# hhergeth/CudaTracerLib

Measured on AMD Instinct MI355X. Metric: Mrays/s at 1920x1080, 267 spp (steps), depth-8; achieved HBM GB/s vs peak, higher is better.
Workload: dtype f32; 1 GPU; synthetic-SM 1920x1080, 1 spp/step, depth 8, NEE on, 2000 instances x icosphere(4)/boxes, 8631000 instanced triangles; rough_transmittance=the reference's 3-D lookup on every call (bit-equal frames), framebuffer_reduce=none (1 GPU)

## Files before the change

### cudatracerlib_amd/build.py

```python
import hashlib, os, subprocess, sys, glob, tempfile

HERE = os.path.dirname(os.path.abspath(__file__))
CSRC = os.path.join(HERE, "csrc")
OUT = os.path.join(HERE, "libctl_amd.so")
SRCS = ["kernels.hip", "shade_basic.hip", "shade_full.hip", "shade_class_a.hip", "shade_class_b.hip", "shade_class_c.hip", "shade_class_p.hip", "shade_class_g.hip", "shade_class_g_wf.hip", "shade_class_p_wf.hip", "shade_class_a_wf.hip", "shade_class_b_wf.hip", "shade_class_c_wf.hip", "shade_basic_wf.hip", "shade_full_wf.hip", "shade_full_media.hip", "shade_full_media_grid.hip", "shade_full_partials.hip", "medium_stage.hip", "megakernel.hip", "prim_tracer.hip", "traversal_probe.hip", "shading_eval_basic.hip", "shading_eval_full.hip", "shading_eval_partials.hip", "image_pipeline.hip", "nlm_filter.hip", "block_sampler.hip", "tracer.hip", "scene_update.hip", "flat_refit.hip", "flat_rebuild.hip", "flat_nodes.hip", "flat_meshes.hip", "flat_mesh_set.hip", "mesh_skin.hip", "shape_set.hip", "scene_images.hip", "volume_eval.hip", "capi.hip", "scene_builder.cpp", "scene_checks.cpp", "geometry_hash.cpp", "bvh_builder.cpp", "sbvh_builder.cpp", "flatten.cpp", "flat_rebuild.cpp", "flat_nodes.cpp", "flat_meshes.cpp", "flat_mesh_set.cpp", "mitsuba_loader.cpp", "image_io.cpp", "jpeg_decode.cpp", "mesh_io.cpp", "scene_cache.cpp", "comm.cpp"]
FLAGS = ["-O3", "-std=c++17", "--offload-arch=gfx950", "-fPIC", "-ffp-contract=off", "-munsafe-fp-atomics",
         "-Wall", "-Wno-unused-function", "-Wno-unused-variable", "-pthread",
         "-Xarch_device", "-fno-slp-vectorize"]


KNOBS_OUT = os.path.join(HERE, "libctl_knobs.so")


def _flag_key(defines=()):
    return hashlib.sha256(("\0".join(sorted(defines)) + "\1" + os.environ.get("CTL_BUILD_EXTRA_FLAGS", "")).encode()).hexdigest()[:16]


def _object_dir(out):
    if out is None:
        return os.path.join(HERE, "build")
    return os.path.join(os.environ.get("TMPDIR") or tempfile.gettempdir(), "ctl_build_" + os.path.splitext(os.path.basename(out))[0])


def stale(target=None, defines=()):
# ... 50 lines not shown
```

### cudatracerlib_amd/csrc/device_scene.h

```cpp
#pragma once
#include "../../include/ctl_amd.h"
#include "ctl_math.h"

namespace ctl {

constexpr int kExitMarker = 0x76543211;
enum { kShadeMoreBsdfs = 1, kShadeRoughBsdfs = 2, kShadeImageTextures = 4, kShadeMoreLights = 8, kShadeNestingBsdfs = 16, kShadeSurfaceMaps = 32, kShadeMoreMicrofacet = 64 };
constexpr int kStackSize = 96;

inline bool is_simple_bsdf(uint32_t t) {
    return t == CTL_BSDF_DIFFUSE || t == CTL_BSDF_DIELECTRIC || t == CTL_BSDF_THINDIELECTRIC || t == CTL_BSDF_ROUGHDIELECTRIC || t == CTL_BSDF_CONDUCTOR || t == CTL_BSDF_ROUGHCONDUCTOR ||
           t == CTL_BSDF_PLASTIC || t == CTL_BSDF_PHONG || t == CTL_BSDF_ROUGHDIFFUSE || t == CTL_BSDF_WARD || t == CTL_BSDF_ROUGHPLASTIC;
}
inline int nested_bsdf_count(uint32_t t) { return t == CTL_BSDF_BLEND ? 2 : (t == CTL_BSDF_COATING || t == CTL_BSDF_ROUGHCOATING) ? 1 : 0; }
inline bool is_nesting_bsdf(uint32_t t) { return nested_bsdf_count(t) != 0; }
inline const uint32_t* bsdf_distribution(const ctl_material& m) {
    const uint32_t t = m.bsdf_type;
    if (t == CTL_BSDF_ROUGHPLASTIC) return &m.u[2];
    return (t == CTL_BSDF_ROUGHCONDUCTOR || t == CTL_BSDF_ROUGHDIELECTRIC || t == CTL_BSDF_ROUGHCOATING) ? &m.u[0] : nullptr;
}
inline bool bsdf_reads_rough_transmittance(uint32_t t) { return t == CTL_BSDF_ROUGHPLASTIC || t == CTL_BSDF_ROUGHCOATING; }
inline uint32_t bsdf_shade_features(const ctl_material& m) {
    const uint32_t t = m.bsdf_type;
    uint32_t f = 0;
// ... 62 lines not shown
    const float* rt_reduced;
    int start_node;
    uint32_t n_nodes;
    uint32_t num_lights;
    uint32_t env_map_index;
    uint32_t n_lights_buf, n_anim_bytes, n_materials_probe;
    uint32_t alpha_maps;
    uint32_t shade_features;
    uint32_t shade_models;
    float eps;
    uint32_t light_indices[CTL_MAX_NUM_LIGHTS];
    float light_cdf[CTL_MAX_NUM_LIGHTS];
    dev_sensor cam;
};

}
```

### cudatracerlib_amd/csrc/kernels.h

```cpp
#pragma once
#include "device_scene.h"
#include "block_sampler.h"
#include <hip/hip_runtime.h>

namespace ctl {

namespace vol { struct table; }

struct path_soa {
    float4* ray_o;
    float4* ray_d;
    float4* thr;
    float4* rad;
    float4* nor;
    float4* pend;
    float2* px;
    float4* mrec;
};
enum { kFlagSpecular = 1 };
constexpr int kHitConsumed = -2;
constexpr uint32_t kNoShadow = 0xffffffffu;

struct final_soa {
    float4* rad;
// ... 29 lines not shown
    uint32_t n_local_pixels;
    int direct, max_path_length, rr_start_depth;
    int key_from_traversal;
    int model_classes;
    const unsigned char* block_counts;
    uint32_t max_block_count;
    int wavefront_rules;
    int u16_bary;
    float* debug_out; uint32_t debug_x, debug_y;
    float* depth_buffer; uint32_t depth_w, depth_h; float depth_near, depth_far;
    float4* stage; size_t stage_stride;
    float4* stray_stage;
    int tex_partials;
};

struct launch_ctx { hipStream_t stream; int grid_blocks; bool alpha_test = false; };

void launch_sequence_fill(hipStream_t stream, const uint32_t* jumps, const void* starts, uint32_t n_passes, float* t1, float* t2);

void apply_tuning_from_env();
void launch_raygen(const launch_ctx& lc, const dev_scene& S, const wave_queues& Q, const pass_params& P);
void launch_intersect_closest(const launch_ctx& lc, const dev_scene& S, const float4* ro, const float4* rd, const uint32_t* n_ptr, uint32_t* work, float4* hit, int* hit_node);
void launch_intersect_any(const launch_ctx& lc, const dev_scene& S, const float4* ro, const float4* rd, const uint32_t* n_ptr, uint32_t* work, uint32_t* occ, float4* hit = nullptr, int* hit_node = nullptr);
void launch_intersect_pair(const launch_ctx& lc, const dev_scene& S, const float4* ro, const float4* rd, const uint32_t* n_ptr, uint32_t* work, float4* hit, int* hit_node,
                           const float4* sro, const float4* srd, const uint32_t* sn_ptr, uint32_t* swork, uint32_t* occ);
void launch_intersect_count(const launch_ctx& lc, const dev_scene& S, const float4* ro, const float4* rd, const uint32_t* n_ptr, uint32_t* work, float4* hit, int* hit_node,
                            uint32_t* occ, int any_hit, unsigned long long* counts3);
void launch_shade(const launch_ctx& lc, const dev_scene& S, const wave_queues& Q, const pass_params& P, int depth, ctl_pixel_data* image, const vol::table* media = nullptr);
void read_stack_histogram(unsigned long long* h, bool reset);
#define CTL_SHADE_BUILDS(X) \
    X(basic, 0u) X(full, 0u) \
    X(class_a, 0u) X(class_b, CTL_CLASS_B_KEYS) X(class_g, CTL_CLASS_G_KEYS) X(class_p, CTL_CLASS_P_KEYS) X(class_c, CTL_CLASS_C_KEYS)
using shade_launch = void(const launch_ctx& lc, const dev_scene& S, const wave_queues& Q, const pass_params& P, int depth, ctl_pixel_data* image);
#define CTL_SHADE_DECLARE(name, keys) shade_launch launch_shade_##name, launch_shade_##name##_wf;
CTL_SHADE_BUILDS(CTL_SHADE_DECLARE)
#undef CTL_SHADE_DECLARE
using shade_media_launch = void(const launch_ctx& lc, const dev_scene& S, const wave_queues& Q, const pass_params& P, const vol::table& V, int depth, ctl_pixel_data* image);
// ... 26 lines not shown
```

### cudatracerlib_amd/csrc/kernels.hip

```cpp
#include "kernels.h"
#include "traverse.h"
#include "traverse_flat.h"
#include "traverse_flat8.h"
#include "knobs.h"
#include <stdexcept>
#include <type_traits>
#include "shading.h"
#include "compaction.h"
#include "volume.h"
#include <cstdlib>

namespace ctl {

__global__ __launch_bounds__(kWideBlock) void k_raygen(dev_scene S, wave_queues Q, pass_params P) {
    __shared__ uint32_t s_cnt[3][kWideBlock / 64]; __shared__ uint32_t s_base[3];
    const uint32_t tiles_x = (P.width + 63) / 64;
    const uint32_t n_total = P.n_local_pixels * P.batch;
    const uint32_t n1 = CTL_SAMPLER_NUM_SEQUENCES * CTL_SAMPLER_SEQUENCE_LENGTH;
    for (uint32_t gi = blockIdx.x * kWideBlock + threadIdx.x; gi < n_total; gi += gridDim.x * kWideBlock) {
        const uint32_t pass_b = gi / P.n_local_pixels, li = gi - pass_b * P.n_local_pixels;
        uint32_t x, y; const uint32_t tile = tile_order_pixel(tiles_x, P.tile_rank, P.tile_world, li, x, y);
        const uint32_t n_smp = P.block_counts ? P.block_counts[tile] : 1u, max_smp = P.block_counts ? P.max_block_count : 1u;
        for (uint32_t smp = 0; smp < max_smp; smp++) {
        const bool valid = x < P.width && y < P.height && smp < n_smp;
// ... 5 lines not shown
        const f2 pX{ (float)x + j.x, (float)y + j.y };
        const f2 ap = rng.next2();
        f3 o, d; sensor_sample_ray(S.cam, pX, ap, o, d);
        const path_soa& A = Q.path[0];
        A.ray_o[slot] = make_float4(o.x, o.y, o.z, S.eps);
        A.ray_d[slot] = make_float4(d.x, d.y, d.z, 3.402823466e+38f);
        A.thr[slot] = make_float4(1.0f, 1.0f, 1.0f, 0.0f);
        A.rad[slot] = make_float4(0.0f, 0.0f, 0.0f, __uint_as_float(pixel));
        A.nor[slot] = make_float4(0.0f, 0.0f, 0.0f, __uint_as_float(rng.d1 | (rng.d2 << 8) | (pass_b << 16) | (0u << 24)));
        A.pend[slot] = make_float4(0.0f, 0.0f, 0.0f, __uint_as_float(kNoShadow));
        A.px[slot] = make_float2(pX.x, pX.y);
        }
    }
}

#ifndef CTL_INTERSECT_MIN_WAVES
#define CTL_INTERSECT_MIN_WAVES 7
#endif
constexpr int lds_stack_ints(int layout) { return layout == 1 + kFmtQ8 ? (kQ8LdsRows + 1) * 2 * kBlock : (layout ? kFlatLdsRows + 1 : kLdsStack) * kBlock; }
template <bool ANY_HIT, bool COUNT, int LAYOUT, bool ALPHA>
__device__ __forceinline__ void intersect_flat_layout(const dev_scene& S, const float4* __restrict__ ro, const float4* __restrict__ rd, uint32_t n, uint32_t* __restrict__ work, float4* __restrict__ hit, int* __restrict__ hit_node, uint32_t* __restrict__ occ, int* lds_stack, trav_counts& tc) {
    if (LAYOUT == 1 + kFmtQ8) intersect_flat8<ANY_HIT, COUNT, ALPHA>(S, ro, rd, n, work, hit, hit_node, occ, (unsigned long long*)lds_stack, tc);
    else intersect_flat<ANY_HIT, COUNT, ALPHA>(S, ro, rd, n, work, hit, hit_node, occ, lds_stack, tc);
}
template <bool ANY_HIT, bool COUNT, int LAYOUT, bool ALPHA>
#ifdef CTL_INTERSECT_EXACT_WAVES
#define CTL_INTERSECT_WAVES_ATTR __attribute__((amdgpu_waves_per_eu(CTL_INTERSECT_EXACT_WAVES, CTL_INTERSECT_EXACT_WAVES)))
#else
#define CTL_INTERSECT_WAVES_ATTR
#endif
__global__ __launch_bounds__(kBlock, ((LAYOUT && !ALPHA) ? CTL_INTERSECT_MIN_WAVES : 6)) CTL_INTERSECT_WAVES_ATTR void k_intersect(dev_scene S, const float4* __restrict__ ro, const float4* __restrict__ rd, const uint32_t* __restrict__ n_ptr,
                                                       uint32_t* __restrict__ work, float4* __restrict__ hit, int* __restrict__ hit_node, uint32_t* __restrict__ occ,
                                                       unsigned long long* __restrict__ counts3) {
    __shared__ __attribute__((aligned(8))) int lds_stack[lds_stack_ints(LAYOUT)];
    const uint32_t n = *n_ptr;
    trav_counts tc{ 0, 0, 0, 0, 0 };
    if (LAYOUT) intersect_flat_layout<ANY_HIT, COUNT, LAYOUT, ALPHA>(S, ro, rd, n, work, hit, hit_node, occ, lds_stack, tc);
    else intersect_persistent<ANY_HIT, COUNT, ALPHA>(S, ro, rd, n, work, hit, hit_node, occ, lds_stack, tc);
    if (COUNT) {
        atomicAdd(&counts3[0], (unsigned long long)tc.n_inner); atomicAdd(&counts3[1], (unsigned long long)tc.n_tri); atomicAdd(&counts3[2], (unsigned long long)tc.n_inst);
        atomicAdd(&counts3[3], (unsigned long long)tc.w_inner); atomicAdd(&counts3[4], (unsigned long long)tc.w_tri);
    }
}

template <int LAYOUT, bool ALPHA>
// ... 127 lines not shown
    }
}

__global__ __launch_bounds__(kBlock) void k_add_samples(ctl_pixel_data* __restrict__ image, uint32_t W, uint32_t H, uint32_t n, const float* __restrict__ s) {
    for (uint32_t i = blockIdx.x * kBlock + threadIdx.x; i < n; i += gridDim.x * kBlock) add_sample(image, W, H, s[5 * i], s[5 * i + 1], f3(s[5 * i + 2], s[5 * i + 3], s[5 * i + 4]));
}
void launch_add_samples(const launch_ctx& lc, ctl_pixel_data* image, uint32_t W, uint32_t H, uint32_t n, const float* samples5) {
    hipLaunchKernelGGL(k_add_samples, dim3(lc.grid_blocks), dim3(kBlock), 0, lc.stream, image, W, H, n, samples5);
}

void read_stack_histogram(unsigned long long* h, bool reset) {
    if (hipMemcpyFromSymbol(h, HIP_SYMBOL(g_stack_hist), sizeof(unsigned long long) * kStackSize) != hipSuccess) throw std::runtime_error("reading the stack histogram failed");
    if (reset) { unsigned long long z[kStackSize] = {}; if (hipMemcpyToSymbol(HIP_SYMBOL(g_stack_hist), z, sizeof(z)) != hipSuccess) throw std::runtime_error("clearing the stack histogram failed"); }
}
static unsigned g_lds_pad = 0;
static int traversal_blocks(const launch_ctx& lc, int layout, bool alpha) {
    const int cus = lc.grid_blocks / 8, by_regs = (layout && !alpha) ? CTL_INTERSECT_MIN_WAVES : 6;
    const int by_lds = (int)((160u * 1024u) / ((unsigned)sizeof(int) * (unsigned)lds_stack_ints(layout) + g_lds_pad));
    return cus * (by_regs < by_lds ? by_regs : by_lds);
}
void apply_tuning_from_env() {
    static bool done = false;
    if (done) return;
    done = true;
    if (const char* e = knob_env("CTL_LDS_PAD")) { int v = atoi(e); if (v >= 0 && v <= 140000) g_lds_pad = (unsigned)v; }
    if (const char* e = knob_env("CTL_REFILL_IDLE")) { int v = atoi(e); if (v >= 1 && v <= 64) (void)hipMemcpyToSymbol(HIP_SYMBOL(g_refill_idle), &v, sizeof(v)); }
    if (const char* e = knob_env("CTL_CHUNK_GUIDED")) { int v = atoi(e) != 0; (void)hipMemcpyToSymbol(HIP_SYMBOL(g_chunk_guided), &v, sizeof(v)); }
    if (const char* e = knob_env("CTL_LEAF_BATCH")) { int v = atoi(e); if (v >= 1 && v <= 64) (void)hipMemcpyToSymbol(HIP_SYMBOL(g_leaf_batch), &v, sizeof(v)); }
    if (const char* e = knob_env("CTL_LEAF_BATCH_ANY")) { int v = atoi(e); if (v >= 1 && v <= 64) (void)hipMemcpyToSymbol(HIP_SYMBOL(g_leaf_batch_any), &v, sizeof(v)); }
}

void launch_raygen(const launch_ctx& lc, const dev_scene& S, const wave_queues& Q, const pass_params& P) {
    hipLaunchKernelGGL(k_raygen, dim3(lc.grid_blocks / 4), dim3(kWideBlock), 0, lc.stream, S, Q, P);
}
template <class F>
static void with_traversal_kernel(const launch_ctx& lc, const dev_scene& S, F&& f) {
    auto alpha = [&](auto layout) { if (lc.alpha_test) f(layout, std::true_type{}); else f(layout, std::false_type{}); };
    if (!S.flat_nodes) alpha(std::integral_constant<int, 0>{});
    else if (S.flat_format == kFmtQ8) alpha(std::integral_constant<int, 1 + kFmtQ8>{});
    else alpha(std::integral_constant<int, 1 + kFmtQ4>{});
}
template <bool ANY, bool CNT>
static void launch_intersect(const launch_ctx& lc, const dev_scene& S, const float4* ro, const float4* rd, const uint32_t* n_ptr, uint32_t* work, float4* hit, int* hit_node,
                             uint32_t* occ, unsigned long long* counts3) {
    with_traversal_kernel(lc, S, [&](auto layout, auto alpha) {
        constexpr int L = decltype(layout)::value; constexpr bool A = decltype(alpha)::value;
        hipLaunchKernelGGL((k_intersect<ANY, CNT, L, A>), dim3(traversal_blocks(lc, L, A)), dim3(kBlock), g_lds_pad, lc.stream, S, ro, rd, n_ptr, work, hit, hit_node, occ, counts3);
    });
}
void launch_intersect_closest(const launch_ctx& lc, const dev_scene& S, const float4* ro, const float4* rd, const uint32_t* n_ptr, uint32_t* work, float4* hit, int* hit_node) {
    launch_intersect<false, false>(lc, S, ro, rd, n_ptr, work, hit, hit_node, nullptr, nullptr);
}
void launch_intersect_any(const launch_ctx& lc, const dev_scene& S, const float4* ro, const float4* rd, const uint32_t* n_ptr, uint32_t* work, uint32_t* occ, float4* hit, int* hit_node) {
    launch_intersect<true, false>(lc, S, ro, rd, n_ptr, work, hit, hit_node, occ, nullptr);
}
void launch_intersect_pair(const launch_ctx& lc, const dev_scene& S, const float4* ro, const float4* rd, const uint32_t* n_ptr, uint32_t* work, float4* hit, int* hit_node,
                           const float4* sro, const float4* srd, const uint32_t* sn_ptr, uint32_t* swork, uint32_t* occ) {
    with_traversal_kernel(lc, S, [&](auto layout, auto alpha) {
        constexpr int L = decltype(layout)::value; constexpr bool A = decltype(alpha)::value;
        hipLaunchKernelGGL((k_intersect_pair<L, A>), dim3(traversal_blocks(lc, L, A)), dim3(kBlock), g_lds_pad, lc.stream, S, ro, rd, n_ptr, work, hit, hit_node, sro, srd, sn_ptr, swork, occ);
    });
}
void launch_intersect_count(const launch_ctx& lc, const dev_scene& S, const float4* ro, const float4* rd, const uint32_t* n_ptr, uint32_t* work, float4* hit, int* hit_node,
                            uint32_t* occ, int any_hit, unsigned long long* counts3) {
    if (any_hit) launch_intersect<true, true>(lc, S, ro, rd, n_ptr, work, hit, hit_node, occ, counts3);
    else launch_intersect<false, true>(lc, S, ro, rd, n_ptr, work, hit, hit_node, nullptr, counts3);
// ... 80 lines not shown
```

### cudatracerlib_amd/csrc/tracer.h

```cpp
#pragma once
#include "../../include/ctl_amd.h"
#include "device_scene.h"
#include "kernels.h"
#include "sequence_generator.h"
#include "block_sampler.h"
#include "flatten.h"
#include <hip/hip_runtime.h>
#include <map>
#include <set>
#include <string>
#include <vector>
#include <memory>
#include <stdexcept>
#include <climits>

namespace ctl {

struct hip_error : std::runtime_error { using std::runtime_error::runtime_error; };
void throw_hip(hipError_t e, const char* file, int line);
#define CTL_HIP(x) do { hipError_t _e = (x); if (_e != hipSuccess) ::ctl::throw_hip(_e, __FILE__, __LINE__); } while (0)

template <typename T> struct dbuf {
    T* p = nullptr; size_t n = 0;
    dbuf() {}
// ... 265 lines not shown
    void check_media(const Scene* s) const;
    void check_texture_filtering() const;
    void setDepthBuffer(float* device_data, unsigned int dw, unsigned int dh) override { depth_buffer_ = device_data; depth_w_ = dw; depth_h_ = dh; }
    void reservePasses(unsigned int n) override { const unsigned int b = std::min(passBatch(), std::max(1u, n)); growBatch(b, "reservePasses"); ensureTableRing(b); if (w != 0xffffffffu) (void)ensureStage(b); }
protected:
    void DoRender(Image* I, const float* d_t1, const float* d_t2, unsigned int n_batch) override;
    void takeRayCounts(uint64_t& path_rays, uint64_t& shadow_rays_) override;
    unsigned int passBatch() const override;
    bool updatesVarianceInBatch(unsigned int b) override;
private:
    void growBatch(unsigned int b, const char* who);
    float4* ensureStage(unsigned int b);
    wave_queues Q{};
    uint32_t capacity = 0, n_local_pixels = 0, alloc_batch_ = 1;
    float* depth_buffer_ = nullptr; unsigned int depth_w_ = 0, depth_h_ = 0;
    std::vector<std::unique_ptr<dbuf<float4>>> f4_; dbuf<float2> px_[2]; dbuf<float4> stage_, stray_stage_, mrec_[2]; dbuf<int> hit_node_; dbuf<uint32_t> occ_[2], counts_, work_, class_order_, class_counts_; dbuf<unsigned char> mat_key_; dbuf<unsigned long long> stats_;
    int grid_blocks = 0;
    float4* new_f4(size_t n);
};

class PathTracer : public Tracer<true> {
public:
    PathTracer();
    void Resize(unsigned int w, unsigned int h) override;
    void InitializeScene(Scene* s) override;
protected:
    void DoRender(Image* I, const float* d_t1, const float* d_t2, unsigned int n_batch) override;
    void takeRayCounts(uint64_t& path_rays, uint64_t& shadow_rays_) override;
    void DebugInternal(Image* I, unsigned int x, unsigned int y, const float* d_t1, const float* d_t2, float rgb[3]) override;
private:
    dbuf<float> debug_;
// ... 21 lines not shown
```

### cudatracerlib_amd/csrc/tracer.hip

```cpp
#include "tracer.h"
#include "scene_builder.h"
#include "scene_checks.h"
#include "scene_volumes.h"
#include "flatten.h"
#include "image_io.h"
#include "mitsuba_loader.h"
#include "spline.h"
#include "mip_pyramid.h"
#include "ctl_fmath.h"
#include "knobs.h"
#include <algorithm>
#include <thread>
#include <cctype>
#include <cstring>
#include <cstdlib>
#include <string>

namespace ctl {

void throw_hip(hipError_t e, const char* file, int line) {
    throw hip_error(std::string("In file ") + file + ", line " + std::to_string(line) + " : " + hipGetErrorString(e));
}
int device_count() { int n = 0; if (hipGetDeviceCount(&n) != hipSuccess) return 0; return n; }
void require_device() { if (device_count() <= 0) throw hip_error("no HIP device: the MI355X path tracer has no CPU fallback"); apply_tuning_from_env(); }
// ... 454 lines not shown
    takeRayCounts(intersect_rays, shadow_rays);
    m_uLastNumRaysTraced = intersect_rays + shadow_rays;
    m_fAccRuntime += m_fLastRuntime; m_uAccNumRaysTraced += m_uLastNumRaysTraced;
}
template class Tracer<true>;
template class Tracer<false>;

WavefrontPathTracer::WavefrontPathTracer() {
    m_sParameters.addBool("Direct", true);
    m_sParameters.addInterval("MaxPathLength", 50, 1, INT_MAX);
    m_sParameters.addInterval("RRStartDepth", 5, 1, INT_MAX);
    m_sParameters.addInterval("PassBatch", 0, 0, 128);
    m_sParameters.addBool("AlphaTest", false);
    m_sParameters.addBool("ShadeByModelClass", true);
    m_sParameters.addBool("FuseTraversal", true);
    m_sParameters.addEnum("PathSemantics", 0, { "PathTrace", "Wavefront" });
    m_sParameters.addBool("U16Barycentrics", false);
    m_sParameters.addInterval("OrderedAccumulationMaxMB", 4096, 0, 1 << 20);
    m_sParameters.addBool("ParticipatingMedia", false);
    m_sParameters.addBool("TextureFiltering", false);
    m_sParameters.addBool("OrderedAccumulation", true);
    grid_blocks = persistent_grid_blocks();
}
void WavefrontPathTracer::check_media(const Scene* s) const {
    if (m_sParameters.getValue("ParticipatingMedia") == 0) { if (s) s->refuse_volumes("WavefrontPathTracer"); return; }
    if (m_sParameters.getValue("PathSemantics") == 1)
        throw unsupported_error("WavefrontPathTracer: ParticipatingMedia = true with PathSemantics = Wavefront is not supported: pathIterateKernel has no medium rules; participating media are rendered under PathSemantics = PathTrace");
}
void WavefrontPathTracer::check_texture_filtering() const {
    if (m_sParameters.getValue("TextureFiltering") == 0) return;
// ... 101 lines not shown
    P.t1 = d_t1p; P.t2 = (const float2*)d_t2p;
    P.batch = n_batch;
    P.width = w; P.height = h; P.tile_rank = shard_rank; P.tile_world = shard_world; P.n_local_pixels = n_local_pixels;
    P.direct = direct ? 1 : 0; P.max_path_length = maxPathLength; P.rr_start_depth = rrStart;
    P.block_counts = pass_block_counts_; P.max_block_count = pass_max_block_count_;
    P.wavefront_rules = m_sParameters.getValue("PathSemantics") == 1 ? 1 : 0; P.u16_bary = m_sParameters.getValue("U16Barycentrics") != 0 ? 1 : 0;
    P.tex_partials = (m_sParameters.getValue("TextureFiltering") != 0 && (S.shade_features & kShadeImageTextures)) ? 1 : 0;
    P.depth_buffer = depth_buffer_; P.depth_w = depth_w_; P.depth_h = depth_h_; P.depth_near = m_pScene->near_depth; P.depth_far = m_pScene->far_depth;
    P.stage = nullptr; P.stage_stride = (size_t)n_local_pixels;
    if (!pass_block_counts_) P.stage = ensureStage(n_batch);
    P.stray_stage = (batch_variance_ && P.stage) ? stray_stage_.p : nullptr;
    if (pass_block_counts_ && pass_paths_ > capacity) throw std::runtime_error("ray queue overflow: the block sampler asks for more samples in one pass than the queues hold (DoubleRayBuffer.h:86-89)");
    CTL_HIP(hipMemsetAsync(class_counts_.p, 0, n_class * sizeof(uint32_t), stream));
    CTL_HIP(hipMemsetAsync(counts_.p, 0, n_counts * sizeof(uint32_t), stream));
    CTL_HIP(hipMemsetAsync(work_.p, 0, n_work * sizeof(uint32_t), stream));
    timer.begin(stream, 0); launch_raygen(lc, S, Q, P); timer.end(stream);
    auto shadow_pass = [&](int d) {
        timer.begin(stream, 3);
        if (counting) launch_intersect_count(lc, S, Q.sh_o[d & 1], Q.sh_d[d & 1], &Q.counts[d * 4 + 1], &Q.work[2 * d + 3], nullptr, nullptr, Q.sh_occ[d & 1], 1, Q.stats + 7);
        else launch_intersect_any(lc, S, Q.sh_o[d & 1], Q.sh_d[d & 1], &Q.counts[d * 4 + 1], &Q.work[2 * d + 3], Q.sh_occ[d & 1]);
        timer.end(stream);
        shadow_launches++;
    };
    const bool fuse = !counting && direct && m_sParameters.getValue("FuseTraversal") != 0;
    P.model_classes = (!media && S.shade_features != 0 && m_sParameters.getValue("ShadeByModelClass") != 0) ? 1 : 0;
    dev_scene Sk = S; Sk.hit_key_out = (!media && S.flat_leaf_keys && (S.shade_features == 0 || P.model_classes) && !counting) ? Q.mat_key : nullptr;
    P.key_from_traversal = Sk.hit_key_out ? 1 : 0;
    if (!P.key_from_traversal) P.model_classes = 0;
    if (P.model_classes && !class_order_.p) { class_order_.alloc((size_t)capacity * 5); for (int c = 0; c < 5; c++) Q.class_order[c] = class_order_.p + (size_t)c * capacity; }
    for (int depth = 1; depth <= maxPathLength; depth++) {
// ... 2 lines not shown
            const int d = depth - 1;
            timer.begin(stream, 4);
            launch_intersect_pair(lc, Sk, Q.path[cur].ray_o, Q.path[cur].ray_d, &Q.counts[(depth - 1) * 4 + 0], &Q.work[2 * depth], Q.hit, Q.hit_node,
                                  Q.sh_o[d & 1], Q.sh_d[d & 1], &Q.counts[d * 4 + 1], &Q.work[2 * d + 3], Q.sh_occ[d & 1]);
            timer.end(stream);
            fused_launches++;
            timer.begin(stream, 2);
            launch_finalize(lc, Q, P, depth - 1, I->device());
            if (media) launch_medium_stage(lc, S, Q, P, V, depth, I->device());
            launch_shade(lc, S, Q, P, depth, I->device(), media ? &V : nullptr);
            timer.end(stream);
            continue;
        }
        timer.begin(stream, 1);
        if (counting) launch_intersect_count(lc, S, Q.path[cur].ray_o, Q.path[cur].ray_d, &Q.counts[(depth - 1) * 4 + 0], &Q.work[2 * depth], Q.hit, Q.hit_node, nullptr, 0, Q.stats + 2);
        else launch_intersect_closest(lc, Sk, Q.path[cur].ray_o, Q.path[cur].ray_d, &Q.counts[(depth - 1) * 4 + 0], &Q.work[2 * depth], Q.hit, Q.hit_node);
        timer.end(stream);
        intersect_launches++;
        if (depth > 1 && direct) shadow_pass(depth - 1);
        timer.begin(stream, 2);
        if (depth > 1 && direct) launch_finalize(lc, Q, P, depth - 1, I->device());
        if (media) launch_medium_stage(lc, S, Q, P, V, depth, I->device());
        launch_shade(lc, S, Q, P, depth, I->device(), media ? &V : nullptr);
        timer.end(stream);
    }
    if (direct) {
        shadow_pass(maxPathLength);
        timer.begin(stream, 2); launch_finalize(lc, Q, P, maxPathLength, I->device()); timer.end(stream);
    }
    if (batch_variance_ && !P.stage) throw std::runtime_error("WavefrontPathTracer::DoRender: the batch's variance update needs the stage of the ordered accumulation");
// ... 6 lines not shown
```

### cudatracerlib_amd/csrc/traverse_flat.h

```cpp
#pragma once
#include "traverse.h"
#include "flat_slab.h"

namespace ctl {

enum { kFmtQ4 = 0, kFmtQ8 = 3 };

#ifndef CTL_FLAT_LDS_ROWS
#define CTL_FLAT_LDS_ROWS 23
#endif
constexpr int kFlatLdsRows = CTL_FLAT_LDS_ROWS;
constexpr int kTopCache = 0;
__device__ unsigned long long g_stack_hist[kStackSize];
__device__ int g_leaf_batch = 20;

__device__ int g_leaf_batch_any = 20;
typedef __attribute__((address_space(3))) int flat_stack_lds_word;
struct flat_stack {
    flat_stack_lds_word* lds;
    int ovf[kStackSize - kFlatLdsRows];
    __device__ __forceinline__ int get(int i) const {
        int w = lds[(i < kFlatLdsRows ? i : kFlatLdsRows) * 256];
        if (i >= kFlatLdsRows) w = ovf[i - kFlatLdsRows];
        return w;
// ... 142 lines not shown
        dd[k] = (cmax >= cmin) ? cmin : inf;
    }
    if (!ORDERED) {
        const bool e0 = dd[0] < inf, e1 = dd[1] < inf, e2 = dd[2] < inf, e3 = dd[3] < inf;
        const int f23 = e2 ? c[2] : c[3], f123 = e1 ? c[1] : f23;
        const int o0 = e0 ? c[0] : f123, o1 = e0 ? f123 : (e1 ? f23 : c[3]), o2 = (e0 && e1) ? f23 : c[3];
        c[0] = o0; c[1] = o1; c[2] = o2;
        return (int)e0 + (int)e1 + (int)e2 + (int)e3;
    }
    CTL_CSWAP_PAIR(0, 1) CTL_CSWAP_PAIR(2, 3) CTL_CSWAP_PAIR(0, 2) CTL_CSWAP_PAIR(1, 3) CTL_CSWAP_PAIR(1, 2)
    return dd[3] < inf ? 4 : (dd[2] < inf ? 3 : (dd[1] < inf ? 2 : (dd[0] < inf ? 1 : 0)));
}

#undef CTL_CSWAP_PAIR

template <bool ANY_HIT, bool COUNT, bool ALPHA>
__device__ __forceinline__ void intersect_flat(const dev_scene& S, const float4* __restrict__ ro, const float4* __restrict__ rd, uint32_t n, uint32_t* __restrict__ work,
                                               float4* __restrict__ hit, int* __restrict__ hit_node, uint32_t* __restrict__ occ, int* lds_stack_ints, trav_counts& cnt) {
    const int lane = threadIdx.x & 63;
    __shared__ unsigned int s_hist[COUNT ? kStackSize : 1];
    if (COUNT) { for (int i = threadIdx.x; i < kStackSize; i += blockDim.x) s_hist[i] = 0u; __syncthreads(); }
    const int refill_idle = g_refill_idle, leaf_batch = ANY_HIT ? g_leaf_batch_any : g_leaf_batch;
    const bool compact = S.flat_compact != 0;
    flat_stack st; st.lds = (flat_stack_lds_word*)lds_stack_ints + threadIdx.x;
    bool has_ray = false;
    uint32_t ray_id = 0;
    float ox = 0, oy = 0, oz = 0, dx = 0, dy = 0, dz = 0, tmin = 0;
    ray_cull R{ 0, 0, 0, 0, 0, 0 };
    float ht = 0;
    hit_in_memory sink{ ht, ray_id, hit, hit_node, ANY_HIT ? nullptr : S.hit_key_out };
    int sp = 0, node = kSentinel, pend = -1;
    alpha_cand cand{ 0, 0, 0, 0, 0, 0 }; bool has_cand = false;
    constexpr int kAlphaBatch = 12;
// ... 6 lines not shown
        const unsigned long long idle = __ballot(!has_ray);
        if (idle != 0ull && !exhausted && (__popcll(idle) >= refill_idle || idle == ~0ull)) {
            if (chunk_next >= chunk_end) rc.refill(n, work, lane);
            if (!exhausted) {
                const uint32_t prefix = __builtin_amdgcn_mbcnt_hi((uint32_t)(idle >> 32), __builtin_amdgcn_mbcnt_lo((uint32_t)idle, 0));
                const uint32_t avail = chunk_end - chunk_next, want = (uint32_t)__popcll(idle);
                const uint32_t my = chunk_next + prefix;
                if (!has_ray && prefix < avail) {
                    const float4 o = ro[my], d = rd[my];
                    ray_id = my; has_ray = true;
                    ox = o.x; oy = o.y; oz = o.z; tmin = o.w; dx = d.x; dy = d.y; dz = d.z;
                    R.idx = rcp_cull(dx); R.idy = rcp_cull(dy); R.idz = rcp_cull(dz);
                    R.oox = ox * R.idx; R.ooy = oy * R.idy; R.ooz = oz * R.idz;
                    ht = d.w;
                    sp = 0; st.put_row(0, kSentinel); node = S.flat_root; pend = -1;
                }
                chunk_next += want < avail ? want : avail;
            }
        }
        if (__ballot(has_ray) == 0ull) { if (exhausted) break; continue; }

        if (has_ray && !has_cand && node < 0 && pend < 0) { pend = ~node; node = st.get(sp); sp--; }
        const bool at_inner = has_ray && !has_cand && (unsigned)node < (unsigned)kSentinel;
        const bool at_leaf = has_ray && !has_cand && pend >= 0;
        const unsigned long long m_inner = __ballot(at_inner), m_leaf = __ballot(at_leaf);
        const unsigned long long m_cand = ALPHA ? __ballot(has_cand) : 0ull;
        bool finished = false;
        if (ALPHA && m_cand != 0ull && (__popcll(m_cand) >= kAlphaBatch || (m_inner == 0ull && m_leaf == 0ull))) {
            if (has_cand) {
                has_cand = false;
// ... 90 lines not shown
```

Measured before the change: 3368 Mrays/s.

## Seed primary-ray traversal with per-8x8-tile frustum-culled BVH entry lists

Adds a kernel that, for each 8x8 pixel tile, descends the top levels of the quantized BVH using the tile's camera frustum planes. It records up to eight surviving nodes, sorted by entry distance. A specialised first-bounce intersect kernel then starts each camera ray from its tile's list instead of the root, skipping the shared upper-level node visits. The cost is an extra per-frame kernel, a table read per ray, and conservative culling tolerances that must not drop valid subtrees.

```diff
diff --git a/cudatracerlib_amd/build.py b/cudatracerlib_amd/build.py
--- a/cudatracerlib_amd/build.py
+++ b/cudatracerlib_amd/build.py
@@ -3,7 +3,7 @@
 HERE = os.path.dirname(os.path.abspath(__file__))
 CSRC = os.path.join(HERE, "csrc")
 OUT = os.path.join(HERE, "libctl_amd.so")
-SRCS = ["kernels.hip", "shade_basic.hip", "shade_full.hip", "shade_class_a.hip", "shade_class_b.hip", "shade_class_c.hip", "shade_class_p.hip", "shade_class_g.hip", "shade_class_g_wf.hip", "shade_class_p_wf.hip", "shade_class_a_wf.hip", "shade_class_b_wf.hip", "shade_class_c_wf.hip", "shade_basic_wf.hip", "shade_full_wf.hip", "shade_full_media.hip", "shade_full_media_grid.hip", "shade_full_partials.hip", "medium_stage.hip", "megakernel.hip", "prim_tracer.hip", "traversal_probe.hip", "shading_eval_basic.hip", "shading_eval_full.hip", "shading_eval_partials.hip", "image_pipeline.hip", "nlm_filter.hip", "block_sampler.hip", "tracer.hip", "scene_update.hip", "flat_refit.hip", "flat_rebuild.hip", "flat_nodes.hip", "flat_meshes.hip", "flat_mesh_set.hip", "mesh_skin.hip", "shape_set.hip", "scene_images.hip", "volume_eval.hip", "capi.hip", "scene_builder.cpp", "scene_checks.cpp", "geometry_hash.cpp", "bvh_builder.cpp", "sbvh_builder.cpp", "flatten.cpp", "flat_rebuild.cpp", "flat_nodes.cpp", "flat_meshes.cpp", "flat_mesh_set.cpp", "mitsuba_loader.cpp", "image_io.cpp", "jpeg_decode.cpp", "mesh_io.cpp", "scene_cache.cpp", "comm.cpp"]
+SRCS = ["kernels.hip", "entry_lists.hip","shade_basic.hip", "shade_full.hip", "shade_class_a.hip", "shade_class_b.hip", "shade_class_c.hip", "shade_class_p.hip", "shade_class_g.hip", "shade_class_g_wf.hip", "shade_class_p_wf.hip", "shade_class_a_wf.hip", "shade_class_b_wf.hip", "shade_class_c_wf.hip", "shade_basic_wf.hip", "shade_full_wf.hip", "shade_full_media.hip", "shade_full_media_grid.hip", "shade_full_partials.hip", "medium_stage.hip", "megakernel.hip", "prim_tracer.hip", "traversal_probe.hip", "shading_eval_basic.hip", "shading_eval_full.hip", "shading_eval_partials.hip", "image_pipeline.hip", "nlm_filter.hip", "block_sampler.hip", "tracer.hip", "scene_update.hip", "flat_refit.hip", "flat_rebuild.hip", "flat_nodes.hip", "flat_meshes.hip", "flat_mesh_set.hip", "mesh_skin.hip", "shape_set.hip", "scene_images.hip", "volume_eval.hip", "capi.hip", "scene_builder.cpp", "scene_checks.cpp", "geometry_hash.cpp", "bvh_builder.cpp", "sbvh_builder.cpp", "flatten.cpp", "flat_rebuild.cpp", "flat_nodes.cpp", "flat_meshes.cpp", "flat_mesh_set.cpp", "mitsuba_loader.cpp", "image_io.cpp", "jpeg_decode.cpp", "mesh_io.cpp", "scene_cache.cpp", "comm.cpp"]
 FLAGS = ["-O3", "-std=c++17", "--offload-arch=gfx950", "-fPIC", "-ffp-contract=off", "-munsafe-fp-atomics",
          "-Wall", "-Wno-unused-function", "-Wno-unused-variable", "-pthread",
          "-Xarch_device", "-fno-slp-vectorize"]
diff --git a/cudatracerlib_amd/csrc/device_scene.h b/cudatracerlib_amd/csrc/device_scene.h
--- a/cudatracerlib_amd/csrc/device_scene.h
+++ b/cudatracerlib_amd/csrc/device_scene.h
@@ -100,4 +100,11 @@
     dev_sensor cam;
 };
 
+constexpr int kEntryListCap = 8, kEntryListCut = 5;
+struct entry_lists {
+    const uint32_t* table;
+    const float4* pixel_w;
+    uint32_t width, blocks_x;
+};
+
 }
diff --git a/cudatracerlib_amd/csrc/entry_lists.hip b/cudatracerlib_amd/csrc/entry_lists.hip
--- /dev/null
+++ b/cudatracerlib_amd/csrc/entry_lists.hip
@@ -0,0 +1,103 @@
+#include "kernels.h"
+#include "traverse.h"
+#include "traverse_flat.h"
+#include "shading.h"
+#include "compaction.h"
+#include <stdexcept>
+
+namespace ctl {
+
+__global__ __launch_bounds__(256) void k_entry_lists(dev_scene S, uint32_t blocks_x, uint32_t n_blocks, int cap, uint32_t* __restrict__ table) {
+    const uint32_t b = blockIdx.x * 256u + threadIdx.x;
+    if (b >= n_blocks) return;
+    uint32_t* __restrict__ out = table + (size_t)b * (1 + kEntryListCap);
+    const float x0 = (float)((b % blocks_x) * 8u), y0 = (float)((b / blocks_x) * 8u);
+    f3 eye, c[4], dc;
+    const f2 ap{ 0.5f, 0.5f };
+    sensor_sample_ray(S.cam, f2{ x0, y0 }, ap, eye, c[0]); sensor_sample_ray(S.cam, f2{ x0 + 8.0f, y0 }, ap, eye, c[1]);
+    sensor_sample_ray(S.cam, f2{ x0 + 8.0f, y0 + 8.0f }, ap, eye, c[2]); sensor_sample_ray(S.cam, f2{ x0, y0 + 8.0f }, ap, eye, c[3]);
+    sensor_sample_ray(S.cam, f2{ x0 + 4.0f, y0 + 4.0f }, ap, eye, dc);
+    const f3 mid = c[0] + c[1] + c[2] + c[3];
+    f3 pn[4]; bool ok = true;
+    for (int i = 0; i < 4; i++) {
+        f3 nrm = cross(c[i], c[(i + 1) & 3]);
+        const float len = length(nrm);
+        if (!(len > 0.0f) || !(len < __builtin_huge_valf())) ok = false;
+        nrm = nrm * (1.0f / len);
+        pn[i] = dot(nrm, mid) < 0.0f ? -nrm : nrm;
+    }
+    if (!ok) { out[0] = 0u; return; }
+    const float tiny = 1e-30f;
+    const f3 idc(1.0f / (fabsf(dc.x) > tiny ? dc.x : copysign_bits(tiny, dc.x)), 1.0f / (fabsf(dc.y) > tiny ? dc.y : copysign_bits(tiny, dc.y)), 1.0f / (fabsf(dc.z) > tiny ? dc.z : copysign_bits(tiny, dc.z)));
+
+    int link[kEntryListCap], dep[kEntryListCap], n = 1; float tn[kEntryListCap];
+    link[0] = S.flat_root; dep[0] = 0; tn[0] = 0.0f;
+    for (;;) {
+        int j = -1;
+        for (int i = 0; i < n; i++) if (link[i] >= 0 && dep[i] < kEntryListCut) { j = i; break; }
+        if (j < 0) break;
+        const float4* __restrict__ p = S.flat_nodes + (link[j] & ~3);
+        const float4 q0 = p[0], q1 = p[1], q2 = p[2];
+        const uint32_t meta = __float_as_uint(q0.w), w0 = __float_as_uint(q2.z), w1 = __float_as_uint(q2.w);
+        const uint32_t ib4 = w0 & 0x03fffffcu, nlb15 = (w1 >> 6) | 0xfc000000u, leafm = meta >> 28;
+        const uint32_t t4[4] = { 0u, (w0 >> 26) & 15u, (w1 >> 2) & 15u, (w0 >> 30) | ((w1 & 3u) << 2) };
+        const float sx = __uint_as_float((meta & 0xffu) << 23), sy = __uint_as_float(((meta >> 8) & 0xffu) << 23), sz = __uint_as_float(((meta >> 16) & 0xffu) << 23);
+        const uint32_t bl[3] = { __float_as_uint(q1.x), __float_as_uint(q1.z), __float_as_uint(q2.x) }, bh[3] = { __float_as_uint(q1.y), __float_as_uint(q1.w), __float_as_uint(q2.y) };
+        int kl[4]; float kt[4]; int nk = 0;
+        for (int k = 0; k < 4; k++) {
+            if (!((meta >> (24 + k)) & 1u)) continue;
+            const f3 lo(__builtin_fmaf((float)((bl[0] >> (8 * k)) & 0xffu), sx, q0.x), __builtin_fmaf((float)((bl[1] >> (8 * k)) & 0xffu), sy, q0.y), __builtin_fmaf((float)((bl[2] >> (8 * k)) & 0xffu), sz, q0.z));
+            const f3 hi(__builtin_fmaf((float)((bh[0] >> (8 * k)) & 0xffu), sx, q0.x), __builtin_fmaf((float)((bh[1] >> (8 * k)) & 0xffu), sy, q0.y), __builtin_fmaf((float)((bh[2] >> (8 * k)) & 0xffu), sz, q0.z));
+            if (!(lo.x <= hi.x && lo.y <= hi.y && lo.z <= hi.z)) continue;
+            bool inside = true;
+            for (int i = 0; i < 4; i++) {
+                const f3 far((pn[i].x > 0.0f ? hi.x : lo.x) - eye.x, (pn[i].y > 0.0f ? hi.y : lo.y) - eye.y, (pn[i].z > 0.0f ? hi.z : lo.z) - eye.z);
+                const float tol = 2e-5f * (fabsf(far.x) + fabsf(far.y) + fabsf(far.z)) + 4.0f * (sx + sy + sz) * 1.1920929e-7f + tiny;
+                if (dot(pn[i], far) < -tol) inside = false;
+            }
+            if (!inside) continue;
+            const f3 a = (lo - eye) * idc, e = (hi - eye) * idc;
+            kt[nk] = max2(max2(max2(min2(a.x, e.x), min2(a.y, e.y)), min2(a.z, e.z)), 0.0f);
+            kl[nk] = k == 0 ? ((leafm & 1u) ? (int)(nlb15 + 15u) : (int)(w0 & 0x03ffffffu)) : (int)((((leafm >> k) & 1u) ? nlb15 : ib4) + t4[k]);
+            nk++;
+        }
+        if (n - 1 + nk > cap) break;
+        const int d1 = dep[j] + 1;
+        for (int i = j; i + 1 < n; i++) { link[i] = link[i + 1]; dep[i] = dep[i + 1]; tn[i] = tn[i + 1]; }
+        n--;
+        for (int k = 0; k < nk; k++) { link[n] = kl[k]; dep[n] = d1; tn[n] = kt[k]; n++; }
+    }
+    if (n == 0) { out[0] = 1u; out[1] = (uint32_t)kSentinel; return; }
+    for (int i = 1; i < n; i++) {
+        const int l = link[i]; const float t = tn[i]; int m = i;
+        while (m > 0 && tn[m - 1] > t) { link[m] = link[m - 1]; tn[m] = tn[m - 1]; m--; }
+        link[m] = l; tn[m] = t;
+    }
+    out[0] = (uint32_t)n;
+    for (int i = 0; i < kEntryListCap; i++) out[1 + i] = (uint32_t)(i < n ? link[i] : kSentinel);
+}
+
+void launch_entry_lists(const launch_ctx& lc, const dev_scene& S, uint32_t width, uint32_t height, uint32_t cap, uint32_t* table) {
+    const uint32_t bx = (width + 7u) / 8u, by = (height + 7u) / 8u, n = bx * by;
+    if (!n) return;
+    const int c = (int)(cap < 1u ? 1u : (cap > (uint32_t)kEntryListCap ? (uint32_t)kEntryListCap : cap));
+    hipLaunchKernelGGL(k_entry_lists, dim3((n + 255u) / 256u), dim3(256), 0, lc.stream, S, bx, n, c, table);
+}
+
+__global__ __launch_bounds__(kBlock, CTL_INTERSECT_MIN_WAVES) CTL_INTERSECT_WAVES_ATTR void k_intersect_first(dev_scene S, const float4* __restrict__ ro, const float4* __restrict__ rd, const uint32_t* __restrict__ n_ptr,
+                                                                                                                  uint32_t* __restrict__ work, float4* __restrict__ hit, int* __restrict__ hit_node, entry_lists EL) {
+    __shared__ __attribute__((aligned(8))) int lds_stack[(kFlatLdsRows + 1) * kBlock]   ;
+    trav_counts tc{ 0, 0, 0, 0, 0 };
+    intersect_flat<false, false, false, true>(S, ro, rd, *n_ptr, work, hit, hit_node, nullptr, lds_stack, tc, EL);
+}
+void launch_intersect_first(const launch_ctx& lc, const dev_scene& S, const float4* ro, const float4* rd, const uint32_t* n_ptr, uint32_t* work, float4* hit, int* hit_node, const entry_lists& EL) {
+    if (!entry_lists_apply(lc, S) || !EL.table) throw std::runtime_error("launch_intersect_first: the scene takes no entry lists");
+    hipLaunchKernelGGL(k_intersect_first, dim3(traversal_blocks(lc, 1 + kFmtQ4, false)), dim3(kBlock), traversal_lds_pad(), lc.stream, S, ro, rd, n_ptr, work, hit, hit_node, EL);
+}
+void apply_first_bounce_tuning(int refill_idle, int chunk_guided, int leaf_batch) {
+    if (refill_idle >= 0) (void)hipMemcpyToSymbol(HIP_SYMBOL(g_refill_idle), &refill_idle, sizeof(int));
+    if (chunk_guided >= 0) (void)hipMemcpyToSymbol(HIP_SYMBOL(g_chunk_guided), &chunk_guided, sizeof(int));
+    if (leaf_batch >= 0) (void)hipMemcpyToSymbol(HIP_SYMBOL(g_leaf_batch), &leaf_batch, sizeof(int));
+}
+
+}
diff --git a/cudatracerlib_amd/csrc/kernels.h b/cudatracerlib_amd/csrc/kernels.h
--- a/cudatracerlib_amd/csrc/kernels.h
+++ b/cudatracerlib_amd/csrc/kernels.h
@@ -67,6 +67,15 @@
     int tex_partials;
 };
 
+#ifndef CTL_INTERSECT_MIN_WAVES
+#define CTL_INTERSECT_MIN_WAVES 7
+#endif
+#ifdef CTL_INTERSECT_EXACT_WAVES
+#define CTL_INTERSECT_WAVES_ATTR __attribute__((amdgpu_waves_per_eu(CTL_INTERSECT_EXACT_WAVES, CTL_INTERSECT_EXACT_WAVES)))
+#else
+#define CTL_INTERSECT_WAVES_ATTR
+#endif
+
 struct launch_ctx { hipStream_t stream; int grid_blocks; bool alpha_test = false; };
 
 void launch_sequence_fill(hipStream_t stream, const uint32_t* jumps, const void* starts, uint32_t n_passes, float* t1, float* t2);
@@ -74,6 +83,12 @@
 void apply_tuning_from_env();
 void launch_raygen(const launch_ctx& lc, const dev_scene& S, const wave_queues& Q, const pass_params& P);
 void launch_intersect_closest(const launch_ctx& lc, const dev_scene& S, const float4* ro, const float4* rd, const uint32_t* n_ptr, uint32_t* work, float4* hit, int* hit_node);
+bool entry_lists_apply(const launch_ctx& lc, const dev_scene& S);
+int traversal_blocks(const launch_ctx& lc, int layout, bool alpha);
+unsigned traversal_lds_pad();
+void apply_first_bounce_tuning(int refill_idle, int chunk_guided, int leaf_batch);
+void launch_entry_lists(const launch_ctx& lc, const dev_scene& S, uint32_t width, uint32_t height, uint32_t cap, uint32_t* table);
+void launch_intersect_first(const launch_ctx& lc, const dev_scene& S, const float4* ro, const float4* rd, const uint32_t* n_ptr, uint32_t* work, float4* hit, int* hit_node, const entry_lists& EL);
 void launch_intersect_any(const launch_ctx& lc, const dev_scene& S, const float4* ro, const float4* rd, const uint32_t* n_ptr, uint32_t* work, uint32_t* occ, float4* hit = nullptr, int* hit_node = nullptr);
 void launch_intersect_pair(const launch_ctx& lc, const dev_scene& S, const float4* ro, const float4* rd, const uint32_t* n_ptr, uint32_t* work, float4* hit, int* hit_node,
                            const float4* sro, const float4* srd, const uint32_t* sn_ptr, uint32_t* swork, uint32_t* occ);
diff --git a/cudatracerlib_amd/csrc/kernels.hip b/cudatracerlib_amd/csrc/kernels.hip
--- a/cudatracerlib_amd/csrc/kernels.hip
+++ b/cudatracerlib_amd/csrc/kernels.hip
@@ -43,9 +43,6 @@
     }
 }
 
-#ifndef CTL_INTERSECT_MIN_WAVES
-#define CTL_INTERSECT_MIN_WAVES 7
-#endif
 constexpr int lds_stack_ints(int layout) { return layout == 1 + kFmtQ8 ? (kQ8LdsRows + 1) * 2 * kBlock : (layout ? kFlatLdsRows + 1 : kLdsStack) * kBlock; }
 template <bool ANY_HIT, bool COUNT, int LAYOUT, bool ALPHA>
 __device__ __forceinline__ void intersect_flat_layout(const dev_scene& S, const float4* __restrict__ ro, const float4* __restrict__ rd, uint32_t n, uint32_t* __restrict__ work, float4* __restrict__ hit, int* __restrict__ hit_node, uint32_t* __restrict__ occ, int* lds_stack, trav_counts& tc) {
@@ -53,11 +50,6 @@
     else intersect_flat<ANY_HIT, COUNT, ALPHA>(S, ro, rd, n, work, hit, hit_node, occ, lds_stack, tc);
 }
 template <bool ANY_HIT, bool COUNT, int LAYOUT, bool ALPHA>
-#ifdef CTL_INTERSECT_EXACT_WAVES
-#define CTL_INTERSECT_WAVES_ATTR __attribute__((amdgpu_waves_per_eu(CTL_INTERSECT_EXACT_WAVES, CTL_INTERSECT_EXACT_WAVES)))
-#else
-#define CTL_INTERSECT_WAVES_ATTR
-#endif
 __global__ __launch_bounds__(kBlock, ((LAYOUT && !ALPHA) ? CTL_INTERSECT_MIN_WAVES : 6)) CTL_INTERSECT_WAVES_ATTR void k_intersect(dev_scene S, const float4* __restrict__ ro, const float4* __restrict__ rd, const uint32_t* __restrict__ n_ptr,
                                                        uint32_t* __restrict__ work, float4* __restrict__ hit, int* __restrict__ hit_node, uint32_t* __restrict__ occ,
                                                        unsigned long long* __restrict__ counts3) {
@@ -215,19 +207,20 @@
     if (reset) { unsigned long long z[kStackSize] = {}; if (hipMemcpyToSymbol(HIP_SYMBOL(g_stack_hist), z, sizeof(z)) != hipSuccess) throw std::runtime_error("clearing the stack histogram failed"); }
 }
 static unsigned g_lds_pad = 0;
-static int traversal_blocks(const launch_ctx& lc, int layout, bool alpha) {
+int traversal_blocks(const launch_ctx& lc, int layout, bool alpha) {
     const int cus = lc.grid_blocks / 8, by_regs = (layout && !alpha) ? CTL_INTERSECT_MIN_WAVES : 6;
     const int by_lds = (int)((160u * 1024u) / ((unsigned)sizeof(int) * (unsigned)lds_stack_ints(layout) + g_lds_pad));
     return cus * (by_regs < by_lds ? by_regs : by_lds);
 }
+unsigned traversal_lds_pad() { return g_lds_pad; }
 void apply_tuning_from_env() {
     static bool done = false;
     if (done) return;
     done = true;
     if (const char* e = knob_env("CTL_LDS_PAD")) { int v = atoi(e); if (v >= 0 && v <= 140000) g_lds_pad = (unsigned)v; }
-    if (const char* e = knob_env("CTL_REFILL_IDLE")) { int v = atoi(e); if (v >= 1 && v <= 64) (void)hipMemcpyToSymbol(HIP_SYMBOL(g_refill_idle), &v, sizeof(v)); }
-    if (const char* e = knob_env("CTL_CHUNK_GUIDED")) { int v = atoi(e) != 0; (void)hipMemcpyToSymbol(HIP_SYMBOL(g_chunk_guided), &v, sizeof(v)); }
-    if (const char* e = knob_env("CTL_LEAF_BATCH")) { int v = atoi(e); if (v >= 1 && v <= 64) (void)hipMemcpyToSymbol(HIP_SYMBOL(g_leaf_batch), &v, sizeof(v)); }
+    if (const char* e = knob_env("CTL_REFILL_IDLE")) { int v = atoi(e); if (v >= 1 && v <= 64) { (void)hipMemcpyToSymbol(HIP_SYMBOL(g_refill_idle), &v, sizeof(v)); apply_first_bounce_tuning(v, -1, -1); } }
+    if (const char* e = knob_env("CTL_CHUNK_GUIDED")) { int v = atoi(e) != 0; (void)hipMemcpyToSymbol(HIP_SYMBOL(g_chunk_guided), &v, sizeof(v)); apply_first_bounce_tuning(-1, v, -1); }
+    if (const char* e = knob_env("CTL_LEAF_BATCH")) { int v = atoi(e); if (v >= 1 && v <= 64) { (void)hipMemcpyToSymbol(HIP_SYMBOL(g_leaf_batch), &v, sizeof(v)); apply_first_bounce_tuning(-1, -1, v); } }
     if (const char* e = knob_env("CTL_LEAF_BATCH_ANY")) { int v = atoi(e); if (v >= 1 && v <= 64) (void)hipMemcpyToSymbol(HIP_SYMBOL(g_leaf_batch_any), &v, sizeof(v)); }
 }
 
@@ -251,6 +244,9 @@
 }
 void launch_intersect_closest(const launch_ctx& lc, const dev_scene& S, const float4* ro, const float4* rd, const uint32_t* n_ptr, uint32_t* work, float4* hit, int* hit_node) {
     launch_intersect<false, false>(lc, S, ro, rd, n_ptr, work, hit, hit_node, nullptr, nullptr);
+}
+bool entry_lists_apply(const launch_ctx& lc, const dev_scene& S) {
+    return S.flat_nodes && S.flat_format == kFmtQ4 && S.flat_compact && !lc.alpha_test && S.cam.type == CTL_SENSOR_PERSPECTIVE;
 }
 void launch_intersect_any(const launch_ctx& lc, const dev_scene& S, const float4* ro, const float4* rd, const uint32_t* n_ptr, uint32_t* work, uint32_t* occ, float4* hit, int* hit_node) {
     launch_intersect<true, false>(lc, S, ro, rd, n_ptr, work, hit, hit_node, occ, nullptr);
diff --git a/cudatracerlib_amd/csrc/tracer.h b/cudatracerlib_amd/csrc/tracer.h
--- a/cudatracerlib_amd/csrc/tracer.h
+++ b/cudatracerlib_amd/csrc/tracer.h
@@ -303,7 +303,7 @@
     wave_queues Q{};
     uint32_t capacity = 0, n_local_pixels = 0, alloc_batch_ = 1;
     float* depth_buffer_ = nullptr; unsigned int depth_w_ = 0, depth_h_ = 0;
-    std::vector<std::unique_ptr<dbuf<float4>>> f4_; dbuf<float2> px_[2]; dbuf<float4> stage_, stray_stage_, mrec_[2]; dbuf<int> hit_node_; dbuf<uint32_t> occ_[2], counts_, work_, class_order_, class_counts_; dbuf<unsigned char> mat_key_; dbuf<unsigned long long> stats_;
+    std::vector<std::unique_ptr<dbuf<float4>>> f4_; dbuf<float2> px_[2]; dbuf<float4> stage_, stray_stage_, mrec_[2]; dbuf<int> hit_node_; dbuf<uint32_t> occ_[2], counts_, work_, class_order_, class_counts_, entry_lists_; dbuf<unsigned char> mat_key_; dbuf<unsigned long long> stats_;
     int grid_blocks = 0;
     float4* new_f4(size_t n);
 };
diff --git a/cudatracerlib_amd/csrc/tracer.hip b/cudatracerlib_amd/csrc/tracer.hip
--- a/cudatracerlib_amd/csrc/tracer.hip
+++ b/cudatracerlib_amd/csrc/tracer.hip
@@ -492,6 +492,8 @@
     m_sParameters.addBool("AlphaTest", false);
     m_sParameters.addBool("ShadeByModelClass", true);
     m_sParameters.addBool("FuseTraversal", true);
+    m_sParameters.addBool("EntryLists", true);
+    m_sParameters.addInterval("EntryListCap", kEntryListCap, 1, kEntryListCap);
     m_sParameters.addEnum("PathSemantics", 0, { "PathTrace", "Wavefront" });
     m_sParameters.addBool("U16Barycentrics", false);
     m_sParameters.addInterval("OrderedAccumulationMaxMB", 4096, 0, 1 << 20);
@@ -623,6 +625,12 @@
     CTL_HIP(hipMemsetAsync(class_counts_.p, 0, n_class * sizeof(uint32_t), stream));
     CTL_HIP(hipMemsetAsync(counts_.p, 0, n_counts * sizeof(uint32_t), stream));
     CTL_HIP(hipMemsetAsync(work_.p, 0, n_work * sizeof(uint32_t), stream));
+    const bool first_lists = !counting && m_sParameters.getValue("EntryLists") != 0 && entry_lists_apply(lc, S);
+    if (first_lists) {
+        const size_t n_words = (size_t)((w + 7u) / 8u) * ((h + 7u) / 8u) * (1 + kEntryListCap);
+        if (entry_lists_.n < n_words) entry_lists_.alloc(n_words);
+        launch_entry_lists(lc, S, w, h, (uint32_t)m_sParameters.getValue("EntryListCap"), entry_lists_.p);
+    }
     timer.begin(stream, 0); launch_raygen(lc, S, Q, P); timer.end(stream);
     auto shadow_pass = [&](int d) {
         timer.begin(stream, 3);
@@ -655,6 +663,7 @@
         }
         timer.begin(stream, 1);
         if (counting) launch_intersect_count(lc, S, Q.path[cur].ray_o, Q.path[cur].ray_d, &Q.counts[(depth - 1) * 4 + 0], &Q.work[2 * depth], Q.hit, Q.hit_node, nullptr, 0, Q.stats + 2);
+        else if (depth == 1 && first_lists) launch_intersect_first(lc, Sk, Q.path[0].ray_o, Q.path[0].ray_d, &Q.counts[0], &Q.work[2], Q.hit, Q.hit_node, entry_lists{ entry_lists_.p, Q.path[0].rad, w, (w + 7u) / 8u });
         else launch_intersect_closest(lc, Sk, Q.path[cur].ray_o, Q.path[cur].ray_d, &Q.counts[(depth - 1) * 4 + 0], &Q.work[2 * depth], Q.hit, Q.hit_node);
         timer.end(stream);
         intersect_launches++;
diff --git a/cudatracerlib_amd/csrc/traverse_flat.h b/cudatracerlib_amd/csrc/traverse_flat.h
--- a/cudatracerlib_amd/csrc/traverse_flat.h
+++ b/cudatracerlib_amd/csrc/traverse_flat.h
@@ -180,9 +180,10 @@
 
 #undef CTL_CSWAP_PAIR
 
-template <bool ANY_HIT, bool COUNT, bool ALPHA>
+template <bool ANY_HIT, bool COUNT, bool ALPHA, bool LISTS = false>
 __device__ __forceinline__ void intersect_flat(const dev_scene& S, const float4* __restrict__ ro, const float4* __restrict__ rd, uint32_t n, uint32_t* __restrict__ work,
-                                               float4* __restrict__ hit, int* __restrict__ hit_node, uint32_t* __restrict__ occ, int* lds_stack_ints, trav_counts& cnt) {
+                                               float4* __restrict__ hit, int* __restrict__ hit_node, uint32_t* __restrict__ occ, int* lds_stack_ints, trav_counts& cnt,
+                                               const entry_lists EL = entry_lists{ nullptr, nullptr, 0u, 0u }) {
     const int lane = threadIdx.x & 63;
     __shared__ unsigned int s_hist[COUNT ? kStackSize : 1];
     if (COUNT) { for (int i = threadIdx.x; i < kStackSize; i += blockDim.x) s_hist[i] = 0u; __syncthreads(); }
@@ -219,6 +220,17 @@
                     R.oox = ox * R.idx; R.ooy = oy * R.idy; R.ooz = oz * R.idz;
                     ht = d.w;
                     sp = 0; st.put_row(0, kSentinel); node = S.flat_root; pend = -1;
+                    if (LISTS) {
+                        const uint32_t pixel = __float_as_uint(EL.pixel_w[my].w), py = pixel / EL.width, px = pixel - py * EL.width;
+                        const uint32_t* __restrict__ L = EL.table + (size_t)((py >> 3) * EL.blocks_x + (px >> 3)) * (1 + kEntryListCap);
+                        const int cnt_l = (int)L[0];
+                        if (cnt_l > 0) {
+                            node = (int)L[1];
+#pragma unroll
+                            for (int i = 2; i <= kEntryListCap; i++) st.put_row(i <= cnt_l ? cnt_l - i + 1 : kFlatLdsRows, (int)L[i]);
+                            sp = cnt_l - 1;
+                        }
+                    }
                 }
                 chunk_next += want < avail ? want : avail;
             }
```

After: 3386 Mrays/s (median of 6 runs). No clear change (+0.5%).
